# svenstaro/bvh

Measured on AMD Instinct MI355X. Metric: Mrays/s (build+traverse), higher is better.
Workload: dtype f32; 1 GPU; configs[1]: create_n_cubes(10000), 120000 triangles f32/3D, 1000000 create_ray rays per GPU; step = build_par+flatten+traverse; triangles=120000, rays_per_gpu=1000000, rays_total=1000000, scene_dist=single, flat_array=eager, parallelism=rays sharded x1

## Files before the change

### bvh_amd/csrc/traverse.hip

```cpp
#include <cstdio>
#include <type_traits>

#include "point_dist.hpp"
#include "walk.hpp"

namespace bvhgpu {

template <typename T, int MODE, bool STATS>
__global__ __launch_bounds__(256) void k_traverse(const TravNode<T>* __restrict__ nodes, uint32_t n_trav,
                                                  const typename Traits<T>::Ray* __restrict__ rays, uint32_t n_rays,
                                                  WalkOut<T> w) {
    const uint32_t r = blockIdx.x * blockDim.x + threadIdx.x;
    const int lane = lane_id();
    const unsigned long long lt = lanemask_lt();
    const bool active = r < n_rays;
    LaneRay<T, MODE> ray;
    ray.clear();
    if (active) ray.load(rays, r, w.tmax);
    uint32_t i = active ? 0u : n_trav;
    PoolCursor pc;
    unsigned long long steps = 0, leaf_steps = 0, wsteps = 0;
    const bool fast = MODE != MODE_T_SLICE && !__any(active && !ray.fin);
    while (true) {
        const bool run = i < n_trav;
// ... 118 lines not shown
    __device__ __forceinline__ void put(uint32_t e, T d, uint32_t n) {
        if (e < HEAP_LDS) { sd[e][tid] = d; sn[e][tid] = n; }
        else { gd[(size_t)(e - HEAP_LDS) * G + g] = d; gn[(size_t)(e - HEAP_LDS) * G + g] = n; }
    }
    __device__ __forceinline__ void sift_up(uint32_t pos, T d, uint32_t n) {
        while (pos > 0) {
            const uint32_t parent = (pos - 1) >> 1;
            const T pd = dist(parent);
            if (d <= pd) break;
            put(pos, pd, node(parent));
            pos = parent;
        }
        put(pos, d, n);
    }
};

template <typename T, int MODE, bool ASCENDING>
__global__ __launch_bounds__(256) void k_traverse_heap(const typename Traits<T>::Node* __restrict__ nodes, uint32_t n_nodes,
                                                       const T* __restrict__ shape_aabbs,
                                                       const typename Traits<T>::Ray* __restrict__ rays, uint32_t n_rays,
                                                       WalkOut<T> w, T* __restrict__ heap_dist, uint32_t* __restrict__ heap_node,
                                                       uint32_t heap_cap, uint32_t* __restrict__ overflow) {
    __shared__ T s_dist[HEAP_LDS][256];
    __shared__ uint32_t s_node[HEAP_LDS][256];
    const int lane = lane_id();
    const unsigned long long lt = lanemask_lt();
    LaneHeap<T> hp;
    hp.sd = s_dist; hp.sn = s_node; hp.gd = heap_dist; hp.gn = heap_node;
    hp.G = (size_t)gridDim.x * 256; hp.g = (size_t)blockIdx.x * 256 + threadIdx.x; hp.tid = threadIdx.x;
    const uint32_t cap = HEAP_LDS + heap_cap;
    PoolCursor pc;
    bool ovf = false;
    LaneRay<T, MODE> ray;
    for (size_t base = (size_t)blockIdx.x * 256; base < n_rays; base += hp.G) {
        const size_t r = base + threadIdx.x;
        const bool active = r < n_rays;
        ray.clear();
        if (active) ray.load(rays, (uint32_t)r);
        uint32_t len = 0;
        if (active && n_nodes) {
            bool has_node = true;
            const uint32_t rs = nodes[0].shape;
            if (rs != NONE) {
                const T* sb = shape_aabbs + 6 * (size_t)rs;
                const T mn[3] = {sb[0], sb[1], sb[2]}, mx[3] = {sb[3], sb[4], sb[5]};
                T t0, t1;
                has_node = slab_hit<T>(ray.o, ray.inv, mn, mx, t0, t1);
            }
            if (has_node) { hp.put(0, ASCENDING ? -(T)0 : (T)0, 0u); len = 1; }
        }
        while (true) {
            const bool run = len > 0;
            if (!__any(run)) break;
            bool rec = false;
            uint32_t shape = NONE;
            if (run) {
                len--;
                const T last_d = hp.dist(len);
                uint32_t node_index = hp.node(len);
                if (len > 0) {
                    const uint32_t last_n = node_index;
                    node_index = hp.node(0);
                    uint32_t pos = 0, child = 1;
                    while (child + 1 < len) {
                        T cd = hp.dist(child);
                        const T cr = hp.dist(child + 1);
                        if (cd <= cr) { child++; cd = cr; }
                        hp.put(pos, cd, hp.node(child));
                        pos = child;
                        child = 2 * pos + 1;
                    }
                    if (child == len - 1) { hp.put(pos, hp.dist(child), hp.node(child)); pos = child; }
                    hp.sift_up(pos, last_d, last_n);
                }
                const typename Traits<T>::Node* nd = nodes + node_index;
                const uint32_t ns = nd->shape;
                if (ns != NONE) {
                    rec = true; shape = ns;
                } else {
                    T lmn[3], lmx[3], rmn[3], rmx[3];
#pragma unroll
                    for (int k = 0; k < 3; k++) { lmn[k] = nd->l_min[k]; lmx[k] = nd->l_max[k]; rmn[k] = nd->r_min[k]; rmx[k] = nd->r_max[k]; }
                    const uint32_t li = nd->l, ri = nd->r;
                    T l0, l1, r0, r1;
                    const bool lh = slab_hit<T>(ray.o, ray.inv, lmn, lmx, l0, l1);
                    const bool rh = slab_hit<T>(ray.o, ray.inv, rmn, rmx, r0, r1);
                    if (len + (lh ? 1u : 0u) + (rh ? 1u : 0u) > cap) {
                        ovf = true; len = 0;
                    } else {
                        if (lh) { hp.sift_up(len, ASCENDING ? -l0 : l1, li); len++; }
                        if (rh) { hp.sift_up(len, ASCENDING ? -r0 : r1, ri); len++; }
                    }
                }
            }
            report<T, MODE>(rec, shape, (T)0, (T)0, ray, w, pc, lane, lt);
        }
        if (active) ray.retire(w);
    }
    if (ovf) atomicOr(overflow, HEAP_OVERFLOW_BIT);
    walk_epilogue<T, MODE>(w, pc, lane, false, 0, 0, 0, 0);
}

template <typename T> struct TopLds;
template <> struct TopLds<float> {
    static constexpr uint32_t BYTES_PER_SLOT = 32;
    float4 *lo, *hi;
    __device__ __forceinline__ TopLds(unsigned char* base, uint32_t K) {
        lo = reinterpret_cast<float4*>(base); hi = lo + K;
    }
    __device__ __forceinline__ void store(uint32_t q, const TravNode<float>* g) {
        const float4* p = reinterpret_cast<const float4*>(g);
        lo[q] = p[0]; hi[q] = p[1];
    }
    __device__ __forceinline__ NodeRegs<float> load(uint32_t q) const {
        const float4 a = lo[q], b = hi[q];
        NodeRegs<float> r;
        r.mn[0] = a.x; r.mn[1] = a.y; r.mn[2] = a.z; r.exit = __float_as_uint(a.w);
        r.mx[0] = b.x; r.mx[1] = b.y; r.mx[2] = b.z; r.shape = __float_as_uint(b.w);
        return r;
    }
};
template <> struct TopLds<double> {
    static constexpr uint32_t BYTES_PER_SLOT = 56;
    double2 *a, *b, *c;
    uint2* d;
    __device__ __forceinline__ TopLds(unsigned char* base, uint32_t K) {
        a = reinterpret_cast<double2*>(base); b = a + K; c = b + K; d = reinterpret_cast<uint2*>(c + K);
    }
    __device__ __forceinline__ void store(uint32_t q, const TravNode<double>* g) {
        const double2* p = reinterpret_cast<const double2*>(g);
        a[q] = p[0]; b[q] = p[1]; c[q] = p[2];
        const unsigned long long es = (unsigned long long)__double_as_longlong(p[3].x);
        d[q] = make_uint2((uint32_t)(es & 0xFFFFFFFFull), (uint32_t)(es >> 32));
    }
    __device__ __forceinline__ NodeRegs<double> load(uint32_t q) const {
        const double2 x = a[q], y = b[q], z = c[q];
        const uint2 w = d[q];
        NodeRegs<double> r;
        r.mn[0] = x.x; r.mn[1] = x.y; r.mn[2] = y.x;
        r.mx[0] = y.y; r.mx[1] = z.x; r.mx[2] = z.y;
        r.exit = w.x; r.shape = w.y;
        return r;
    }
};

constexpr int LDS_THREADS = 1024;
#ifndef BVH_LDS_INNER
#define BVH_LDS_INNER 8
#endif
constexpr int LDS_INNER = BVH_LDS_INNER;

template <typename T, int MODE, bool STATS>
__global__ __launch_bounds__(LDS_THREADS) void k_traverse_lds(const TravNode<T>* __restrict__ nodes, uint32_t n_trav,
                                                               const uint32_t* __restrict__ slot_entry, uint32_t K,
                                                               uint32_t first_slot, uint32_t split,
                                                               const typename Traits<T>::Ray* __restrict__ rays,
                                                               uint32_t n_rays, uint32_t rays_per_wg, WalkOut<T> w) {
    extern __shared__ __attribute__((aligned(16))) unsigned char smem[];
    uint32_t& s_next = *reinterpret_cast<uint32_t*>(smem);
    TopLds<T> top(smem + 16, K);
    const uint32_t split_at = split ? load_node(nodes).exit : 0u;
    const unsigned long long g0 = (unsigned long long)blockIdx.x * rays_per_wg;
    const unsigned long long g1 = g0 + rays_per_wg;
    const uint32_t wg_begin = (uint32_t)(g0 < n_rays ? g0 : n_rays);
    const uint32_t wg_end = (uint32_t)(g1 < n_rays ? g1 : n_rays);
    if (threadIdx.x == 0) s_next = wg_begin;
    for (uint32_t q = threadIdx.x; q < K; q += blockDim.x) {
        const uint32_t e = slot_entry[q];
        if (e != NONE) top.store(q, nodes + e);
    }
    __syncthreads();

    const int lane = lane_id();
    const unsigned long long lt = lanemask_lt();
    LaneRay<T, MODE> ray;
    ray.clear();
    uint32_t i = 0, limit = 0, slot = SLOT_NONE;
    bool exhausted = wg_begin >= wg_end;
    PoolCursor pc;
    unsigned long long steps = 0, leaf_steps = 0, wsteps = 0, cands = 0;
    while (true) {
        bool run = i < limit;
        const unsigned long long idle = __ballot(!run);
        if (idle) {
            if (!run && ray.r != NONE) { cands += ray.cnt; ray.retire(w); }
            if (!exhausted) {
                const uint32_t nidle = (uint32_t)__popcll(idle);
                uint32_t base = 0;
                if (lane == 0) base = atomicAdd(&s_next, nidle);
                base = __builtin_amdgcn_readfirstlane(base);
                const uint32_t mine = base + (uint32_t)__popcll(idle & lt);
                if (!run && base < wg_end && mine < wg_end) {
                    if (split_at) {
                        const bool right = (mine & 1u) != 0u;
                        ray.load(rays, mine >> 1, w.tmax);
                        ray.r = mine;
                        i = right ? split_at : 0u; limit = right ? n_trav : split_at;
                        slot = right ? 3u : 2u;
                    } else {
                        ray.load(rays, mine, w.tmax);
                        i = 0; limit = n_trav; slot = first_slot;
                    }
                    run = true;
                }
                exhausted = base >= wg_end || (wg_end - base) <= nidle;
            }
            if (!__any(run)) break;
        }
        const bool fast = MODE != MODE_T_SLICE && !__any(run && !ray.fin);
        for (int s = 0; s < LDS_INNER; s++) {
            bool rec = false;
            uint32_t shape = NONE;
            T t0 = 0, t1 = 0;
            if (STATS) wsteps++;
            if (i < limit) {
                NodeRegs<T> nd;
                if (slot < K) nd = top.load(slot);
                else nd = load_node(nodes + i);
                const bool hit = fast ? slab_hit_finite<T>(ray.o, ray.inv, nd.mn, nd.mx)
                                      : slab_hit<T>(ray.o, ray.inv, nd.mn, nd.mx, t0, t1);
                shape = nd.shape;
                const bool leaf = trav_is_leaf(shape);
                rec = hit && leaf;
                const bool descend = hit && !leaf;
                i = descend ? i + 1 : nd.exit;
                const uint32_t child = min(slot << 1, SLOT_NONE);
                slot = descend ? child : (leaf ? SLOT_NONE : (shape & 0xFFFFu));
                if (STATS) { steps++; leaf_steps += leaf ? 1 : 0; }
            }
            report<T, MODE>(rec, shape, t0, t1, ray, w, pc, lane, lt);
            if (MODE == MODE_ANY && ray.best_prim != NONE) i = limit;
        }
    }
    walk_epilogue<T, MODE>(w, pc, lane, STATS, steps, leaf_steps, wsteps, cands);
}

constexpr uint32_t CUR_NONE = 0x7FFFFFFFu;
#ifndef BVH_WIDE_INNER_STEPS
#define BVH_WIDE_INNER_STEPS 4
#endif
#ifndef BVH_WIDE_INNER_STEPS_WHOLE
#define BVH_WIDE_INNER_STEPS_WHOLE 8
#endif
#ifndef BVH_WIDE_INNER_STEPS_COHERENT
#define BVH_WIDE_INNER_STEPS_COHERENT 12
#endif
#ifndef BVH_WIDE_MIN_WAVES_F32
#define BVH_WIDE_MIN_WAVES_F32 8
#endif
#ifndef BVH_WIDE_MIN_WAVES_F64
#define BVH_WIDE_MIN_WAVES_F64 4
#endif
constexpr uint32_t WIDE_ITEM_BITS = 5;
constexpr uint32_t WIDE_ITEM_WHOLE = 16;
constexpr uint32_t WIDE_BSUM_MAX = 128;
constexpr size_t WIDE_ITEM_MAX_RAYS = (size_t)1 << 27;


__device__ __forceinline__ uint32_t wide_resident_ref(uint32_t ref, uint32_t q, uint32_t c, uint32_t K) {
    const uint32_t cs = 4u * q + 1u + c;
    return (ref != NONE && (ref & WIDE_INNER) && cs < K) ? (WIDE_INNER | WIDE_RESIDENT | cs) : ref;
}

template <typename T, bool EXACT>
__device__ __forceinline__ uint32_t wide_hits(const T o[3], const T inv[3], const WideRegs<T>& nd) {
    uint32_t m = 0;
    if (!EXACT) {
#pragma unroll
        for (int c = 0; c < 4; c++) {
            const T mn[3] = {nd.mn[0][c], nd.mn[1][c], nd.mn[2][c]}, mx[3] = {nd.mx[0][c], nd.mx[1][c], nd.mx[2][c]};
            m |= slab_hit_finite<T>(o, inv, mn, mx) ? (1u << c) : 0u;
        }
        return m;
    }
#pragma unroll
    for (int p = 0; p < 2; p++) {
        const int c0 = 2 * p, c1 = 2 * p + 1;
        const T mn0[3] = {nd.mn[0][c0], nd.mn[1][c0], nd.mn[2][c0]}, mx0[3] = {nd.mx[0][c0], nd.mx[1][c0], nd.mx[2][c0]};
        T t0, t1;
        if (nd.ref[c1] == NONE) {
            if (nd.ref[c0] != NONE && slab_hit<T>(o, inv, mn0, mx0, t0, t1)) m |= 1u << c0;
        } else {
            const T mn1[3] = {nd.mn[0][c1], nd.mn[1][c1], nd.mn[2][c1]}, mx1[3] = {nd.mx[0][c1], nd.mx[1][c1], nd.mx[2][c1]};
            T jmn[3], jmx[3];
#pragma unroll
            for (int k = 0; k < 3; k++) { jmn[k] = tmin(mn0[k], mn1[k]); jmx[k] = tmax(mx0[k], mx1[k]); }
            if (slab_hit<T>(o, inv, jmn, jmx, t0, t1)) {
                if (slab_hit<T>(o, inv, mn0, mx0, t0, t1)) m |= 1u << c0;
                if (slab_hit<T>(o, inv, mn1, mx1, t0, t1)) m |= 1u << c1;
            }
        }
    }
    return m;
}

#ifndef BVH_WIDE_LONG_FRAC
#define BVH_WIDE_LONG_FRAC 0.2
#endif
template <typename T> struct ItemTable {
    T box[16][6];
    uint32_t ref[16];
    T half_diag[16];
};
template <typename T, int ITEMS_LOG4>
__device__ __forceinline__ void item_table_build(const WideNode<T>* __restrict__ wide, ItemTable<T>* tb, uint32_t tid) {
    constexpr uint32_t ITEMS = 1u << (2 * ITEMS_LOG4);
    if (tid < ITEMS) {
        const uint32_t c = ITEMS_LOG4 == 2 ? tid >> 2 : tid, k = tid & 3u;
        const WideNode<T>* root = wide;
        uint32_t ref = root->ref[c];
        T b[6];
#pragma unroll
        for (int a = 0; a < 3; a++) { b[a] = root->mn[a][c]; b[3 + a] = root->mx[a][c]; }
        if (ITEMS_LOG4 == 2) {
            if (ref != NONE && (ref & WIDE_INNER)) {
                const WideNode<T>* g = wide + (ref & (WIDE_RESIDENT - 1u));
                ref = g->ref[k];
#pragma unroll
                for (int a = 0; a < 3; a++) { b[a] = g->mn[a][k]; b[3 + a] = g->mx[a][k]; }
            } else if (k != 0) {
                ref = NONE;
            }
        }
        if (ref == NONE) {
            const T nan = __builtin_nan("");
#pragma unroll
            for (int a = 0; a < 6; a++) b[a] = nan;
        }
#pragma unroll
        for (int a = 0; a < 6; a++) tb->box[tid][a] = b[a];
        tb->ref[tid] = ref;
        const T dx = b[3] - b[0], dy = b[4] - b[1], dz = b[5] - b[2];
        tb->half_diag[tid] = (T)BVH_WIDE_LONG_FRAC * sqrt(dx * dx + dy * dy + dz * dz);
    }
}
template <int ITEMS_LOG4> __device__ __forceinline__ uint32_t item_slot(uint32_t j) {
    return ITEMS_LOG4 == 2 ? 5u + j : 1u + j;
}

struct GuideArgs;
__device__ __forceinline__ void guide_ray_load(const bvhgpu_ray_f64* __restrict__ rays64, uint32_t r, double S, float o[3], float inv[3], bool& bad);
template <typename T, int L4, bool GUIDE = false>
__device__ __forceinline__ void filter_rays_into_list(const ItemTable<T>* tb, const typename Traits<T>::Ray* __restrict__ rays, uint32_t n_rays,
                                                      uint32_t* __restrict__ list, uint32_t per_wg, uint32_t my_rays, uint32_t G, uint32_t b,
                                                      uint32_t tid, uint32_t bd, int lane, uint32_t* s_nlist, uint32_t* s_nback,
                                                      const bvhgpu_ray_f64* __restrict__ rays64 = nullptr, double guide_S = 0.0, bool* any_bad = nullptr) {
    constexpr uint32_t ITEMS = 1u << (2 * L4);
    for (uint32_t l0 = 0; l0 < my_rays; l0 += bd) {
        const uint32_t local = l0 + tid;
        const uint32_t r = local < my_rays ? ((((local >> 6) * G + b) << 6) | (local & 63u)) : n_rays;
        uint32_t mask = 0, longm = 0;
        if (r < n_rays) {
            T o[3], inv[3];
            if constexpr (GUIDE) {
                bool bad;
                guide_ray_load(rays64, r, guide_S, o, inv, bad);
                *any_bad = *any_bad || bad;
            } else {
                const typename Traits<T>::Ray* rp = rays + r;
#pragma unroll
                for (int k = 0; k < 3; k++) { o[k] = rp->o[k]; inv[k] = rp->inv[k]; }
            }
            if (!ray_is_finite<T>(o, inv)) {
                mask = 1u << WIDE_ITEM_WHOLE; longm = mask;
            } else {
#pragma unroll 4
                for (uint32_t j = 0; j < ITEMS; j++) {
                    const T mn[3] = {tb->box[j][0], tb->box[j][1], tb->box[j][2]}, mx[3] = {tb->box[j][3], tb->box[j][4], tb->box[j][5]};
                    T len;
                    const bool hit = slab_hit_finite_len<T>(o, inv, mn, mx, len);
                    mask |= hit ? (1u << j) : 0u;
                    longm |= (hit && len > tb->half_diag[j]) ? (1u << j) : 0u;
                }
            }
        }
        const uint32_t cap = per_wg * ITEMS;
#pragma unroll
        for (int side = 0; side < 2; side++) {
            const uint32_t mm0 = side ? (mask & ~longm) : (mask & longm);
            const uint32_t mine = (uint32_t)__popc(mm0);
            uint32_t incl = mine;
#pragma unroll
            for (int d = 1; d < WAVE; d <<= 1) {
                const uint32_t u = __shfl_up(incl, d);
                if (lane >= d) incl += u;
            }
            const uint32_t total = __shfl(incl, WAVE - 1);
            uint32_t base = 0;
            if (lane == 0 && total) base = atomicAdd(side ? s_nback : s_nlist, total);
            base = __shfl(base, 0) + incl - mine;
            uint32_t mm = mm0;
            while (mm) {
                const uint32_t bit = (uint32_t)__ffs(mm) - 1u;
                mm &= mm - 1u;
                list[side ? cap - 1u - base : base] = (r << WIDE_ITEM_BITS) | bit;
                base++;
            }
        }
    }
}

template <typename T>
__global__ __launch_bounds__(256) void k_wide_items(const typename Traits<T>::Node* __restrict__ nodes, uint32_t n_nodes,
                                                    const uint32_t* __restrict__ node_count, const uint32_t* __restrict__ build_ctr,
                                                    const typename Traits<T>::Ray* __restrict__ rays, uint32_t n_rays,
                                                    uint32_t* __restrict__ list_all, uint32_t* __restrict__ wg_items) {
    constexpr int L4 = 2;
    constexpr uint32_t ITEMS = 16;
    __shared__ ItemTable<T> tb;
    __shared__ uint32_t s_nlist, s_nback, s_bad;
    const uint32_t tid = threadIdx.x, bd = blockDim.x;
    const int lane = lane_id();
    if (tid == 0) { s_nlist = 0u; s_nback = 0u; s_bad = (build_ctr[BUILD_CTR_TOPMASK] & 0xFFFEu) == 0xFFFEu ? 0u : 1u; }
    __syncthreads();
    if (s_bad) { if (tid == 0) wg_items[2u * blockIdx.x] = NONE; return; }
    if (tid < ITEMS) {
        uint32_t node = 0;
        T bx[6];
        bool ok = n_nodes > 1u;
        uint32_t cnt = ok ? node_count[0] : 0u;
#pragma unroll
        for (int lv = 3; lv >= 0 && ok; lv--) {
            const typename Traits<T>::Node nd = nodes[node];
            const uint32_t right = ((16u + tid) >> lv) & 1u;
            ok = nd.shape == NONE && nd.l < n_nodes && nd.r < n_nodes && nd.r > nd.l;
            if (!ok) break;
            const uint32_t nl = (nd.r - nd.l + 1u) >> 1;
            cnt = right ? cnt - nl : nl;
            node = right ? nd.r : nd.l;
#pragma unroll
            for (int k = 0; k < 3; k++) { bx[k] = right ? nd.r_min[k] : nd.l_min[k]; bx[3 + k] = right ? nd.r_max[k] : nd.l_max[k]; }
        }
        ok = ok && cnt > 1u;
        if (!ok) atomicOr(&s_bad, 1u);
#pragma unroll
        for (int k = 0; k < 6; k++) tb.box[tid][k] = bx[k];
        const T dx = bx[3] - bx[0], dy = bx[4] - bx[1], dz = bx[5] - bx[2];
        tb.half_diag[tid] = (T)BVH_WIDE_LONG_FRAC * sqrt(dx * dx + dy * dy + dz * dz);
    }
    __syncthreads();
    if (s_bad) { if (tid == 0) wg_items[2u * blockIdx.x] = NONE; return; }
    const uint32_t n_blocks = (n_rays + 63u) >> 6;
    const uint32_t my_blocks = n_blocks > blockIdx.x ? (n_blocks - blockIdx.x + gridDim.x - 1u) / gridDim.x : 0u;
    const uint32_t per_wg = ((n_blocks + gridDim.x - 1u) / gridDim.x) << 6;
    uint32_t* list = list_all + (size_t)blockIdx.x * per_wg * ITEMS;
    filter_rays_into_list<T, L4>(&tb, rays, n_rays, list, per_wg, my_blocks << 6, gridDim.x, blockIdx.x, tid, bd, lane, &s_nlist, &s_nback);
    __syncthreads();
    if (tid == 0) { wg_items[2u * blockIdx.x] = s_nlist; wg_items[2u * blockIdx.x + 1u] = s_nback; }
}

constexpr unsigned long long WALK_FLAG_GUIDE_RANGE = 16ull;
struct GuideArgs { const bvhgpu_ray_f64* rays64; const double* aabbs64; const float* info; const double* tris64; };
__device__ __forceinline__ void guide_ray_load(const bvhgpu_ray_f64* __restrict__ rays64, uint32_t r, double S, float o[3], float inv[3], bool& bad) {
    const bvhgpu_ray_f64* q = rays64 + r;
    bad = !(S >= GUIDE_SCENE_MIN) || !(S <= GUIDE_SCENE_MAX);
#pragma unroll
    for (int k = 0; k < 3; k++) {
        const double ok = q->o[k], ik = q->inv[k];
        const double ao = fabs(ok), ainv = fabs(ik), ai = ainv * (4.0 * S);
        bad = bad || !(ao <= GUIDE_ORIGIN_MAX * S) || !(ao <= GUIDE_F32_MAX) || !(ai <= 0x1p100) || !(ai >= 0x1p-100) ||
              !(ainv <= GUIDE_F32_MAX) || !(ainv >= GUIDE_F32_MIN_NORMAL);
        o[k] = (float)ok; inv[k] = (float)ik;
    }
}
__device__ __forceinline__ bool guide_leaf_hit(const GuideArgs& ga, uint32_t ray, uint32_t shape) {
    const bvhgpu_ray_f64* rp = ga.rays64 + ray;
    const double* b = ga.aabbs64 + 6 * (size_t)shape;
    const double o[3] = {rp->o[0], rp->o[1], rp->o[2]}, inv[3] = {rp->inv[0], rp->inv[1], rp->inv[2]};
    const double mn[3] = {b[0], b[1], b[2]}, mx[3] = {b[3], b[4], b[5]};
    return slab_hit_finite<double>(o, inv, mn, mx);
}

#ifndef BVH_GUIDE_CANDIDATE_ATTR
#define BVH_GUIDE_CANDIDATE_ATTR __forceinline__
#endif
__device__ BVH_GUIDE_CANDIDATE_ATTR double guide_candidate_distance(const bvhgpu_ray_f64* __restrict__ rays64, const double* __restrict__ tris64, uint32_t ray, uint32_t shape) {
    const bvhgpu_ray_f64* rp = rays64 + ray;
    const double o[3] = {rp->o[0], rp->o[1], rp->o[2]}, d[3] = {rp->d[0], rp->d[1], rp->d[2]};
    double out[3];
    ray_triangle<double>(o, d, tris64 + 9 * (size_t)shape, out);
    return out[0];
}

#ifdef BVH_WIDE_PROFILE
__device__ unsigned long long g_wide_prof[4 * 16384];
__device__ unsigned long long g_wide_util[16 * 16384];
#endif
template <typename T, int MODE, int ITEMS_LOG4, int MAX_THREADS, int MIN_WAVES, int GUIDE = 0>
__global__ __launch_bounds__(MAX_THREADS, MIN_WAVES) void k_traverse_wide(
    const WideNode<T>* __restrict__ wide, const uint32_t* __restrict__ wslot_node, uint32_t K, uint32_t stack_lds,
    const typename Traits<T>::Ray* __restrict__ rays, uint32_t n_rays, uint32_t* __restrict__ list_all, const uint32_t* __restrict__ wg_items,
    WalkOut<T> w, uint32_t* __restrict__ gstack, uint32_t gstack_cap, uint32_t* __restrict__ overflow, GuideArgs ga, uint32_t whole_steps) {
    static_assert(GUIDE == 0 || ((MODE == MODE_INDICES || MODE == MODE_CLOSEST) && sizeof(T) == 4), "the guide walk is the f32 walk of an f64 index / closest-hit batch");
    constexpr bool GUIDE_CLOSEST = GUIDE != 0 && MODE == MODE_CLOSEST;
    double gbest = 0.0;
    static_assert(ITEMS_LOG4 >= 0 && ITEMS_LOG4 <= 2, "1, 4 or 16 items per ray");
    static_assert(MODE != MODE_T_SLICE, "the t-slice output walks the binary array");
    constexpr int CH = WideIo<T>::CHUNKS;
    constexpr int L4 = ITEMS_LOG4 > 0 ? ITEMS_LOG4 : 1;
    constexpr uint32_t ITEMS = 1u << (2 * L4);
    extern __shared__ __attribute__((aligned(16))) uint4 wsmem[];
    uint32_t& s_next = *reinterpret_cast<uint32_t*>(wsmem);
    uint32_t& s_nlist = *(reinterpret_cast<uint32_t*>(wsmem) + 1);
    uint32_t& s_nback = *(reinterpret_cast<uint32_t*>(wsmem) + 2);
    uint32_t* s_item_ref = reinterpret_cast<uint32_t*>(wsmem + 1);
    uint4* nodes = wsmem + 5;
    uint32_t* s_stack = reinterpret_cast<uint32_t*>(nodes + (size_t)CH * K);
    const uint32_t bd = blockDim.x, tid = threadIdx.x;
    const int WIDE_INNER_STEPS = ITEMS_LOG4 == 0 ? (int)whole_steps : BVH_WIDE_INNER_STEPS;
    constexpr uint32_t SB = MAX_THREADS;
    const size_t G = (size_t)gridDim.x * bd, gid = (size_t)blockIdx.x * bd + tid;
    const int lane = lane_id();
    const unsigned long long lt = lanemask_lt();
    double guide_S = 0.0;
    bool guide_bad = false;
    if constexpr (GUIDE != 0) guide_S = (double)ga.info[0];
#ifdef BVH_WIDE_PROFILE
    const unsigned long long prof_t0 = wall_clock64();
    unsigned long long prof_steps = 0;
    unsigned long long pu[16];
    for (int i = 0; i < 16; i++) pu[i] = 0;
    uint32_t pl_boxes = 0, pl_nohit = 0;
#endif
    const uint32_t n_blocks = (n_rays + 63u) >> 6;
    const uint32_t my_blocks = n_blocks > blockIdx.x ? (n_blocks - blockIdx.x + gridDim.x - 1u) / gridDim.x : 0u;
    const uint32_t per_wg = ((n_blocks + gridDim.x - 1u) / gridDim.x) << 6;
    const uint32_t my_rays = my_blocks << 6;
    auto ray_of = [&](uint32_t local) -> uint32_t { return (((local >> 6) * gridDim.x + blockIdx.x) << 6) | (local & 63u); };
    __shared__ uint32_t s_bsum[WIDE_BSUM_MAX];
    if (w.scan_sums) for (uint32_t b = tid; b < WIDE_BSUM_MAX; b += bd) s_bsum[b] = 0u;
    if (tid == 0) { s_next = 0u; s_nlist = 0u; s_nback = 0u; }
    for (uint32_t q = tid; q < K; q += bd) {
        const uint32_t node = wslot_node[q];
        if (node != NONE) {
            const uint4* src = reinterpret_cast<const uint4*>(wide + node);
            uint4* dst = nodes + (size_t)q * CH;
#pragma unroll
            for (int c = 0; c < CH - 1; c++) dst[c] = src[c];
            uint4 rf = src[CH - 1];
            rf.x = wide_resident_ref(rf.x, q, 0u, K); rf.y = wide_resident_ref(rf.y, q, 1u, K);
            rf.z = wide_resident_ref(rf.z, q, 2u, K); rf.w = wide_resident_ref(rf.w, q, 3u, K);
            dst[CH - 1] = rf;
        }
    }
    uint32_t* list = nullptr;
    if (ITEMS_LOG4 > 0) {
        __shared__ ItemTable<T> tb;
        item_table_build<T, L4>(wide, &tb, tid);
        __syncthreads();
        if (tid < ITEMS) {
            const uint32_t ref = tb.ref[tid], slot = item_slot<L4>(tid);
            s_item_ref[tid] = (ref != NONE && (ref & WIDE_INNER) && slot < K) ? (WIDE_INNER | WIDE_RESIDENT | slot) : ref;
        }
        list = list_all + (size_t)blockIdx.x * per_wg * ITEMS;
        const uint32_t pre_front = wg_items ? wg_items[2u * blockIdx.x] : NONE;
        if (pre_front != NONE) {
            if (tid == 0) { s_nlist = pre_front; s_nback = wg_items[2u * blockIdx.x + 1u]; }
        } else {
            if constexpr (GUIDE != 0) filter_rays_into_list<T, L4, true>(&tb, rays, n_rays, list, per_wg, my_rays, gridDim.x, blockIdx.x, tid, bd, lane, &s_nlist, &s_nback,
                                                                            ga.rays64, guide_S, &guide_bad);
            else filter_rays_into_list<T, L4>(&tb, rays, n_rays, list, per_wg, my_rays, gridDim.x, blockIdx.x, tid, bd, lane, &s_nlist, &s_nback);
        }
        __threadfence_block();
    }
    __syncthreads();
    const uint32_t wg_begin = 0u;
    const uint32_t n_front = s_nlist;
    const uint32_t wg_end = ITEMS_LOG4 == 0 ? my_rays : n_front + s_nback;
#ifdef BVH_WIDE_PROFILE
    const unsigned long long prof_t1 = wall_clock64();
#endif

    LaneRay<T, MODE> ray;
    ray.clear();
    uint32_t cur = CUR_NONE, sp = 0, item = NONE;
    bool exhausted = wg_begin >= wg_end;
    bool ovf = false;
    uint32_t pair_pend = NONE;
    PoolCursor pc;
    auto push_slow = [&](uint32_t v) {
        if (sp < stack_lds) s_stack[sp * SB + tid] = v;
        else if (sp - stack_lds < gstack_cap) gstack[(size_t)(sp - stack_lds) * G + gid] = v;
        else ovf = true;
        sp++;
    };
    auto pop_or_none = [&]() -> uint32_t {
        if (sp == 0) return CUR_NONE;
        sp--;
        if (sp < stack_lds) return s_stack[sp * SB + tid];
        return sp - stack_lds < gstack_cap ? gstack[(size_t)(sp - stack_lds) * G + gid] : CUR_NONE;
    };
    while (true) {
        bool run = cur != CUR_NONE;
        const unsigned long long idle = __ballot(!run);
        if (idle) {
            if (MODE == MODE_INDICES && ITEMS_LOG4 == 0 && w.pool_pair)
                report_pair(false, !run && item != NONE, 0u, ray, pair_pend, w.pool_pair, w.pool_cap, w.ctr, pc, lane, lt);
            if (!run && item != NONE) {
                if (MODE == MODE_ANY) {
                    if constexpr (ITEMS_LOG4 == 0) {
                        const size_t r = item;
                        w.closest[3 * r] = ray.best[0]; w.closest[3 * r + 1] = ray.best[1]; w.closest[3 * r + 2] = ray.best[2];
                        w.closest_prim[r] = ray.best_prim;
                    } else if (ray.best_prim != NONE) {
                        const uint32_t j = item & ((1u << WIDE_ITEM_BITS) - 1u);
                        const uint32_t jj = j == WIDE_ITEM_WHOLE ? 0u : j;
                        atomicMin(&w.any_key[item >> WIDE_ITEM_BITS], (jj << 28) | ray.best_prim);
                    }
                } else if (MODE == MODE_CLOSEST) {
                    if constexpr (ITEMS_LOG4 == 0) {
                        const size_t r = item;
                        if constexpr (!GUIDE_CLOSEST) { w.closest[3 * r] = ray.best[0]; w.closest[3 * r + 1] = ray.best[1]; w.closest[3 * r + 2] = ray.best[2]; }
                        w.closest_prim[r] = ray.best_prim;
                    } else if (ray.best_prim != NONE) {
                        const uint32_t j = item & ((1u << WIDE_ITEM_BITS) - 1u);
                        const uint32_t jj = j == WIDE_ITEM_WHOLE ? 0u : j;
                        if constexpr (sizeof(T) == 4 && !GUIDE_CLOSEST) {
                            const unsigned long long key = ((unsigned long long)Traits<T>::key(ray.best[0]) << 32) | ((unsigned long long)jj << 28) | (unsigned long long)ray.best_prim;
                            atomicMin(&w.closest_key[item >> WIDE_ITEM_BITS], key);
                        } else {
                            const size_t r = item >> WIDE_ITEM_BITS;
                            w.item_cnt[(r << (2 * ITEMS_LOG4)) + jj] = ray.best_prim;
                            atomicOr(&w.ray_items[r], 1u << jj);
                        }
                    }
                } else if (ray.cnt) {
                    uint32_t r = item;
                    if (ITEMS_LOG4 == 0) {
                        w.counts[item] = ray.cnt;
                    } else {
                        const uint32_t j = item & ((1u << WIDE_ITEM_BITS) - 1u);
                        const uint32_t jj = j == WIDE_ITEM_WHOLE ? 0u : j;
                        r = item >> WIDE_ITEM_BITS;
                        atomicAdd(&w.counts[r], ray.cnt);
                        atomicOr(&w.ray_items[r], 1u << jj);
                        w.item_cnt[((size_t)r << (2 * ITEMS_LOG4)) + jj] = ray.cnt;
                    }
                    if (w.scan_sums) atomicAdd(&s_bsum[((r >> 6) - blockIdx.x) / gridDim.x], ray.cnt);
                }
                item = NONE;
            }
            if (!exhausted) {
                const uint32_t nidle = (uint32_t)__popcll(idle);
                uint32_t base = 0;
                if (lane == 0) base = atomicAdd(&s_next, nidle);
                base = __builtin_amdgcn_readfirstlane(base);
                const uint32_t mine = base + (uint32_t)__popcll(idle & lt);
                if (!run && base < wg_end && mine < wg_end) {
                    if (ITEMS_LOG4 == 0) {
                        item = ray_of(mine);
                        if (item < n_rays) {
                            if constexpr (GUIDE != 0) { bool bad; guide_ray_load(ga.rays64, item, guide_S, ray.o, ray.inv, bad); guide_bad = guide_bad || bad; ray.loaded(item); gbest = __builtin_inf(); }
                            else ray.load(rays, item, w.tmax);
                            cur = WIDE_INNER | WIDE_RESIDENT | 0u;
                        } else {
                            item = NONE;
                        }
                    } else {
                        item = list[mine < n_front ? mine : per_wg * ITEMS - 1u - (mine - n_front)];
                        const uint32_t j = item & ((1u << WIDE_ITEM_BITS) - 1u);
                        if constexpr (GUIDE != 0) { bool bad; guide_ray_load(ga.rays64, item >> WIDE_ITEM_BITS, guide_S, ray.o, ray.inv, bad); ray.loaded(item >> WIDE_ITEM_BITS); gbest = __builtin_inf(); }
                        else ray.load(rays, item >> WIDE_ITEM_BITS, w.tmax);
                        cur = j == WIDE_ITEM_WHOLE ? (WIDE_INNER | WIDE_RESIDENT | 0u) : s_item_ref[j];
                        if (j == WIDE_ITEM_WHOLE) item = item & ~((1u << WIDE_ITEM_BITS) - 1u);
                    }
                    ray.r = item;
                    sp = 0;
                    run = cur != CUR_NONE;
                }
                exhausted = base >= wg_end || (wg_end - base) <= nidle;
            }
            if (!__any(run)) break;
        }
        const bool fast = !__any(run && !ray.fin);
#ifdef BVH_WIDE_PROFILE
        prof_steps += WIDE_INNER_STEPS;
        pu[9]++; pu[10] += fast ? 0 : 1;
        pu[8] += WIDE_INNER_STEPS * (unsigned long long)__popcll(__ballot(run));
#endif
        for (int s = 0; s < WIDE_INNER_STEPS; s++) {
#ifdef BVH_WIDE_PROFILE
            {
                const bool in = (cur & WIDE_INNER) != 0u;
                pu[0]++; pu[1] += __popcll(__ballot(in));
                pu[2] += __any(in && (cur & WIDE_RESIDENT)) ? 1 : 0;
                pu[3] += __any(in && !(cur & WIDE_RESIDENT)) ? 1 : 0;
                const bool slow = in && sp + 3u > stack_lds;
                pu[4] += __any(slow) ? 1 : 0; pu[5] += __popcll(__ballot(slow));
                const bool lf = !in && cur < CUR_NONE;
                pu[6] += __popcll(__ballot(lf)); pu[7] += __any(lf) ? 1 : 0;
                pu[11] += __any((in || lf) && sp > stack_lds) ? 1 : 0;
            }
#endif
            if (cur & WIDE_INNER) {
                const uint32_t id = cur & (WIDE_RESIDENT - 1u);
                WideRegs<T> nd;
                if (cur & WIDE_RESIDENT) nd = WideIo<T>::from_lds(nodes, id);
                else nd = WideIo<T>::from_global(wide + id);
                const uint32_t m = fast ? wide_hits<T, false>(ray.o, ray.inv, nd) : wide_hits<T, true>(ray.o, ray.inv, nd);
                const uint32_t first = m & (0u - m);
                const uint32_t rest = m ^ first;
#ifdef BVH_WIDE_PROFILE
                pl_boxes += (uint32_t)__popc(m); pl_nohit += m == 0u ? 1u : 0u;
#endif
                const uint32_t s0 = (rest & 8u) ? nd.ref[3] : ((rest & 4u) ? nd.ref[2] : nd.ref[1]);
                const uint32_t s1 = ((rest & 12u) == 12u) ? nd.ref[2] : nd.ref[1];
                if (sp + 3u <= stack_lds) {
                    uint32_t* at = s_stack + sp * SB + tid;
                    at[0] = s0; at[SB] = s1; at[2 * SB] = nd.ref[1];
                    sp += (uint32_t)__popc(rest);
                } else {
                    if (rest & 8u) push_slow(nd.ref[3]);
                    if (rest & 4u) push_slow(nd.ref[2]);
                    if (rest & 2u) push_slow(nd.ref[1]);
                }
                cur = first == 0u ? pop_or_none() : (first == 1u ? nd.ref[0] : (first == 2u ? nd.ref[1] : (first == 4u ? nd.ref[2] : nd.ref[3])));
            }
            bool rec = cur < CUR_NONE;
            const uint32_t shape = cur;
            if (rec) cur = pop_or_none();
            if (GUIDE) {
                if (__any(rec)) {
                    if (rec) rec = guide_leaf_hit(ga, ITEMS_LOG4 == 0 ? ray.r : (ray.r >> WIDE_ITEM_BITS), shape);
                }
            }
            if (MODE == MODE_INDICES && ITEMS_LOG4 == 0 && w.raybuf) {
                if (rec && (ray.cnt >> w.stage_shift) == 0u) {
                    w.raybuf[((size_t)ray.r << w.stage_shift) | ray.cnt] = shape;
                    ray.cnt++;
                    rec = false;
                }
            }
            if constexpr (GUIDE_CLOSEST) {
                if (__any(rec)) {
                    if (rec) {
                        const double dist = guide_candidate_distance(ga.rays64, ga.tris64, ITEMS_LOG4 == 0 ? ray.r : (ray.r >> WIDE_ITEM_BITS), shape);
                        if (dist < gbest) { gbest = dist; ray.best_prim = shape; }
                        ray.cnt++;
                    }
                }
            } else if (MODE == MODE_INDICES && ITEMS_LOG4 == 0 && w.pool_pair) report_pair(rec, false, shape, ray, pair_pend, w.pool_pair, w.pool_cap, w.ctr, pc, lane, lt);
            else report<T, MODE>(rec, shape, (T)0, (T)0, ray, w, pc, lane, lt);
            if (MODE == MODE_ANY && ray.best_prim != NONE) { cur = CUR_NONE; sp = 0; }
        }
        if (ovf) { cur = CUR_NONE; sp = 0; }
    }
    if (__any(ovf) && lane == 0) atomicOr(overflow, 4u);
    if constexpr (GUIDE != 0) { if (__any(guide_bad) && lane == 0) atomicOr(overflow, (uint32_t)WALK_FLAG_GUIDE_RANGE); }
    if (MODE == MODE_INDICES && ITEMS_LOG4 == 0 && w.pool_pair) {
        pool_invalidate_tail16(w.pool_pair, w.pool_cap, pc, lane);
        pc.left = 0;
    }
    walk_epilogue<T, MODE>(w, pc, lane, false, 0, 0, 0, 0);
    if (MODE < MODE_CLOSEST && w.scan_sums) {
        __syncthreads();
        for (uint32_t b = tid; b < my_blocks; b += bd)
            if (s_bsum[b]) atomicAdd(&w.scan_sums[(b * gridDim.x + blockIdx.x) / (uint32_t)(SCAN_BLOCK / 64)], s_bsum[b]);
    }
#ifdef BVH_WIDE_PROFILE
    if (lane == 0) {
        const size_t wv = gid >> 6;
        if (wv < 16384) {
            g_wide_prof[4 * wv] = prof_t0; g_wide_prof[4 * wv + 1] = prof_t1; g_wide_prof[4 * wv + 2] = wall_clock64(); g_wide_prof[4 * wv + 3] = prof_steps;
            for (int i = 0; i < 12; i++) g_wide_util[16 * wv + i] = pu[i];
            g_wide_util[16 * wv + 12] = 0; g_wide_util[16 * wv + 13] = 0;
        }
    }
    __syncthreads();
    if ((gid >> 6) < 16384) { atomicAdd(&g_wide_util[16 * (gid >> 6) + 12], (unsigned long long)pl_boxes); atomicAdd(&g_wide_util[16 * (gid >> 6) + 13], (unsigned long long)pl_nohit); }
#endif
}


constexpr int COUNT_PLAIN = 0, COUNT_PAIR = 1, COUNT_MASKED = 2;
template <int KIND> __device__ __forceinline__ uint32_t ray_count(const uint32_t* __restrict__ counts, uint32_t r) {
    if (KIND == COUNT_PLAIN || KIND == COUNT_MASKED) return counts[r];
    const uint2 c = reinterpret_cast<const uint2*>(counts)[r];
    return c.x + c.y;
}

template <int KIND>
__global__ __launch_bounds__(256) void k_scan_reduce(const uint32_t* __restrict__ counts, uint32_t n,
                                                     unsigned long long* __restrict__ blocksums) {
    __shared__ unsigned long long ws[4];
    const uint32_t base = blockIdx.x * SCAN_BLOCK + threadIdx.x * SCAN_ITEMS;
    unsigned long long s = 0;
#pragma unroll
    for (int j = 0; j < SCAN_ITEMS; j++) s += (base + j < n) ? ray_count<KIND>(counts, base + j) : 0u;
#pragma unroll
    for (int d = 32; d > 0; d >>= 1) s += __shfl_down(s, d);
    if (lane_id() == 0) ws[threadIdx.x >> 6] = s;
    __syncthreads();
    if (threadIdx.x == 0) blocksums[blockIdx.x] = ws[0] + ws[1] + ws[2] + ws[3];
}

__global__ __launch_bounds__(1024) void k_scan_sums(unsigned long long* __restrict__ blocksums, uint32_t nb,
                                                    unsigned long long* __restrict__ total_out) {
    __shared__ unsigned long long ws[16];
    const uint32_t per = (nb + 1023u) / 1024u;
    const uint32_t lo = min(nb, threadIdx.x * per), hi = min(nb, lo + per);
    unsigned long long s = 0;
    for (uint32_t j = lo; j < hi; j++) s += blocksums[j];
    const int lane = lane_id(), wv = (int)(threadIdx.x >> 6);
    unsigned long long inc = s;
#pragma unroll
    for (int d = 1; d < WAVE; d <<= 1) {
        const unsigned long long u = __shfl_up(inc, d);
        if (lane >= d) inc += u;
    }
    if (lane == WAVE - 1) ws[wv] = inc;
    __syncthreads();
    unsigned long long run = inc - s;
    for (int w2 = 0; w2 < wv; w2++) run += ws[w2];
    for (uint32_t j = lo; j < hi; j++) { const unsigned long long v = blocksums[j]; blocksums[j] = run; run += v; }
    if (threadIdx.x == 1023u) *total_out = run;
}

constexpr uint32_t SCAN_FUSED_MAX_BLOCKS = 2048;

template <int KIND, bool PREFIXED>
__global__ __launch_bounds__(256) void k_scan_final(const uint32_t* __restrict__ counts, uint32_t n,
                                                    const unsigned long long* __restrict__ blocksums,
                                                    unsigned long long* __restrict__ total,
                                                    uint32_t* __restrict__ offsets, uint32_t* __restrict__ ray_items,
                                                    uint16_t* __restrict__ ray_mask, unsigned long long* __restrict__ host_page,
                                                    unsigned long long* __restrict__ other_ctr, const uint32_t* __restrict__ scan_sums,
                                                    uint32_t* __restrict__ other_bsum, uint32_t bsum_cap) {
    __shared__ uint32_t ws[4];
    __shared__ unsigned long long wb[4];
    const uint32_t base = blockIdx.x * SCAN_BLOCK + threadIdx.x * SCAN_ITEMS;
    const int lane = lane_id();
    unsigned long long before = 0;
    if (PREFIXED) {
        before = blocksums[blockIdx.x];
    } else {
        unsigned long long part = 0;
        if (scan_sums) {
            for (uint32_t j = threadIdx.x; j < blockIdx.x; j += 256) part += scan_sums[j];
            if (threadIdx.x == 0) other_bsum[blockIdx.x] = 0u;
            if (blockIdx.x == gridDim.x - 1)
                for (uint32_t j = gridDim.x + threadIdx.x; j < bsum_cap; j += 256) other_bsum[j] = 0u;
        } else {
            for (uint32_t j = threadIdx.x; j < blockIdx.x; j += 256) part += blocksums[j];
        }
#pragma unroll
        for (int d = 32; d > 0; d >>= 1) part += __shfl_down(part, d);
        if (lane == 0) wb[threadIdx.x >> 6] = part;
    }
    uint32_t v[SCAN_ITEMS];
    uint32_t s = 0;
#pragma unroll
    for (int j = 0; j < SCAN_ITEMS; j++) { v[j] = (base + j < n) ? ray_count<KIND>(counts, base + j) : 0u; s += v[j]; }
    if (KIND == COUNT_MASKED) {
#pragma unroll
        for (int j = 0; j < SCAN_ITEMS; j++) {
            if (v[j]) {
                if (ray_items) { ray_mask[base + j] = (uint16_t)ray_items[base + j]; ray_items[base + j] = 0u; }
                const_cast<uint32_t*>(counts)[base + j] = 0u;
            }
        }
    }
    uint32_t inc = s;
#pragma unroll
    for (int d = 1; d < WAVE; d <<= 1) {
// ... 1108 lines not shown
```

Before: 3006 Mrays/s.

## Overlap wide-node image copy, item table loads, and ray prefetch in traversal prologue

Splits the item-table build into separate root and grandchild issue phases and interleaves them with a batched copy of resident wide nodes into the node image. Each thread now holds several uint4 chunks in registers before storing them. The first ray of the filter pass is loaded early, and the filter loop prefetches the next round's ray while processing the current one. The goal is to hide global-memory latency in the kernel prologue, at the cost of more live registers, which may lower occupancy.

```diff
diff --git a/bvh_amd/csrc/traverse.hip b/bvh_amd/csrc/traverse.hip
--- a/bvh_amd/csrc/traverse.hip
+++ b/bvh_amd/csrc/traverse.hip
@@ -444,37 +444,40 @@
     uint32_t ref[16];
     T half_diag[16];
 };
+template <typename T> struct ItemEntry { T b[6]; uint32_t ref; };
 template <typename T, int ITEMS_LOG4>
-__device__ __forceinline__ void item_table_build(const WideNode<T>* __restrict__ wide, ItemTable<T>* tb, uint32_t tid) {
-    constexpr uint32_t ITEMS = 1u << (2 * ITEMS_LOG4);
-    if (tid < ITEMS) {
-        const uint32_t c = ITEMS_LOG4 == 2 ? tid >> 2 : tid, k = tid & 3u;
-        const WideNode<T>* root = wide;
-        uint32_t ref = root->ref[c];
-        T b[6];
-#pragma unroll
-        for (int a = 0; a < 3; a++) { b[a] = root->mn[a][c]; b[3 + a] = root->mx[a][c]; }
-        if (ITEMS_LOG4 == 2) {
-            if (ref != NONE && (ref & WIDE_INNER)) {
-                const WideNode<T>* g = wide + (ref & (WIDE_RESIDENT - 1u));
-                ref = g->ref[k];
-#pragma unroll
-                for (int a = 0; a < 3; a++) { b[a] = g->mn[a][k]; b[3 + a] = g->mx[a][k]; }
-            } else if (k != 0) {
-                ref = NONE;
-            }
-        }
-        if (ref == NONE) {
-            const T nan = __builtin_nan("");
-#pragma unroll
-            for (int a = 0; a < 6; a++) b[a] = nan;
-        }
-#pragma unroll
-        for (int a = 0; a < 6; a++) tb->box[tid][a] = b[a];
-        tb->ref[tid] = ref;
-        const T dx = b[3] - b[0], dy = b[4] - b[1], dz = b[5] - b[2];
-        tb->half_diag[tid] = (T)BVH_WIDE_LONG_FRAC * sqrt(dx * dx + dy * dy + dz * dz);
-    }
+__device__ __forceinline__ void item_table_issue_root(const WideNode<T>* __restrict__ wide, ItemEntry<T>& e, uint32_t tid) {
+    const uint32_t c = ITEMS_LOG4 == 2 ? tid >> 2 : tid;
+    e.ref = wide->ref[c];
+#pragma unroll
+    for (int a = 0; a < 3; a++) { e.b[a] = wide->mn[a][c]; e.b[3 + a] = wide->mx[a][c]; }
+}
+template <typename T, int ITEMS_LOG4>
+__device__ __forceinline__ void item_table_issue_grand(const WideNode<T>* __restrict__ wide, ItemEntry<T>& e, uint32_t tid) {
+    if (ITEMS_LOG4 == 2) {
+        const uint32_t k = tid & 3u;
+        if (e.ref != NONE && (e.ref & WIDE_INNER)) {
+            const WideNode<T>* g = wide + (e.ref & (WIDE_RESIDENT - 1u));
+            e.ref = g->ref[k];
+#pragma unroll
+            for (int a = 0; a < 3; a++) { e.b[a] = g->mn[a][k]; e.b[3 + a] = g->mx[a][k]; }
+        } else if (k != 0) {
+            e.ref = NONE;
+        }
+    }
+}
+template <typename T>
+__device__ __forceinline__ void item_table_store(ItemEntry<T>& e, ItemTable<T>* tb, uint32_t tid) {
+    if (e.ref == NONE) {
+        const T nan = __builtin_nan("");
+#pragma unroll
+        for (int a = 0; a < 6; a++) e.b[a] = nan;
+    }
+#pragma unroll
+    for (int a = 0; a < 6; a++) tb->box[tid][a] = e.b[a];
+    tb->ref[tid] = e.ref;
+    const T dx = e.b[3] - e.b[0], dy = e.b[4] - e.b[1], dz = e.b[5] - e.b[2];
+    tb->half_diag[tid] = (T)BVH_WIDE_LONG_FRAC * sqrt(dx * dx + dy * dy + dz * dz);
 }
 template <int ITEMS_LOG4> __device__ __forceinline__ uint32_t item_slot(uint32_t j) {
     return ITEMS_LOG4 == 2 ? 5u + j : 1u + j;
@@ -482,15 +485,43 @@
 
 struct GuideArgs;
 __device__ __forceinline__ void guide_ray_load(const bvhgpu_ray_f64* __restrict__ rays64, uint32_t r, double S, float o[3], float inv[3], bool& bad);
-template <typename T, int L4, bool GUIDE = false>
+template <typename T> struct FilterRay {
+    T o[3], inv[3];
+    __device__ __forceinline__ void request(const typename Traits<T>::Ray* __restrict__ rays, uint32_t r, uint32_t n_rays) {
+#pragma unroll
+        for (int k = 0; k < 3; k++) { o[k] = 0; inv[k] = 0; }
+        if (r < n_rays) {
+            const typename Traits<T>::Ray* rp = rays + r;
+#pragma unroll
+            for (int k = 0; k < 3; k++) { o[k] = rp->o[k]; inv[k] = rp->inv[k]; }
+        }
+    }
+};
+template <typename T, int L4, bool GUIDE>
 __device__ __forceinline__ void filter_rays_into_list(const ItemTable<T>* tb, const typename Traits<T>::Ray* __restrict__ rays, uint32_t n_rays,
                                                       uint32_t* __restrict__ list, uint32_t per_wg, uint32_t my_rays, uint32_t G, uint32_t b,
                                                       uint32_t tid, uint32_t bd, int lane, uint32_t* s_nlist, uint32_t* s_nback,
-                                                      const bvhgpu_ray_f64* __restrict__ rays64 = nullptr, double guide_S = 0.0, bool* any_bad = nullptr) {
+                                                      const bvhgpu_ray_f64* __restrict__ rays64, double guide_S, bool* any_bad,
+                                                      bool have_first, const FilterRay<T>& first) {
     constexpr uint32_t ITEMS = 1u << (2 * L4);
+    auto ray_of_round = [&](uint32_t l0) -> uint32_t {
+        const uint32_t local = l0 + tid;
+        return local < my_rays ? ((((local >> 6) * G + b) << 6) | (local & 63u)) : n_rays;
+    };
+    FilterRay<T> cur_ray, next_ray;
+    uint32_t r = ray_of_round(0u);
+    if constexpr (!GUIDE) {
+        if (have_first) cur_ray = first;
+        else cur_ray.request(rays, r, n_rays);
+    }
     for (uint32_t l0 = 0; l0 < my_rays; l0 += bd) {
-        const uint32_t local = l0 + tid;
-        const uint32_t r = local < my_rays ? ((((local >> 6) * G + b) << 6) | (local & 63u)) : n_rays;
+        uint32_t r_next = n_rays;
+        if constexpr (!GUIDE) {
+            if (l0 + bd < my_rays) r_next = ray_of_round(l0 + bd);
+            next_ray.request(rays, r_next, n_rays);
+        } else {
+            r = ray_of_round(l0);
+        }
         uint32_t mask = 0, longm = 0;
         if (r < n_rays) {
             T o[3], inv[3];
@@ -499,9 +530,8 @@
                 guide_ray_load(rays64, r, guide_S, o, inv, bad);
                 *any_bad = *any_bad || bad;
             } else {
-                const typename Traits<T>::Ray* rp = rays + r;
-#pragma unroll
-                for (int k = 0; k < 3; k++) { o[k] = rp->o[k]; inv[k] = rp->inv[k]; }
+#pragma unroll
+                for (int k = 0; k < 3; k++) { o[k] = cur_ray.o[k]; inv[k] = cur_ray.inv[k]; }
             }
             if (!ray_is_finite<T>(o, inv)) {
                 mask = 1u << WIDE_ITEM_WHOLE; longm = mask;
@@ -539,7 +569,16 @@
                 base++;
             }
         }
-    }
+        if constexpr (!GUIDE) { r = r_next; cur_ray = next_ray; }
+    }
+}
+template <typename T, int L4>
+__device__ __forceinline__ void filter_rays_into_list(const ItemTable<T>* tb, const typename Traits<T>::Ray* __restrict__ rays, uint32_t n_rays,
+                                                      uint32_t* __restrict__ list, uint32_t per_wg, uint32_t my_rays, uint32_t G, uint32_t b,
+                                                      uint32_t tid, uint32_t bd, int lane, uint32_t* s_nlist, uint32_t* s_nback) {
+    FilterRay<T> none;
+    none.request(rays, n_rays, n_rays);
+    filter_rays_into_list<T, L4, false>(tb, rays, n_rays, list, per_wg, my_rays, G, b, tid, bd, lane, s_nlist, s_nback, nullptr, 0.0, nullptr, false, none);
 }
 
 template <typename T>
@@ -670,38 +709,90 @@
     const uint32_t my_rays = my_blocks << 6;
     auto ray_of = [&](uint32_t local) -> uint32_t { return (((local >> 6) * gridDim.x + blockIdx.x) << 6) | (local & 63u); };
     __shared__ uint32_t s_bsum[WIDE_BSUM_MAX];
+    constexpr bool OWN_ITEMS = ITEMS_LOG4 > 0;
+    const bool ray_first = OWN_ITEMS && GUIDE == 0 && wg_items == nullptr;
+    FilterRay<T> first_ray;
+    first_ray.request(rays, ray_first && tid < my_rays ? ray_of(tid) : n_rays, n_rays);
+    uint32_t pre_front = NONE, pre_back = 0u;
+    if (OWN_ITEMS && wg_items) { pre_front = wg_items[2u * blockIdx.x]; pre_back = wg_items[2u * blockIdx.x + 1u]; }
+    constexpr int IMG = sizeof(T) == 8 ? 8 : 4;
+    const uint32_t img_total = K * (uint32_t)CH;
+    uint32_t img_node[IMG];
+    uint4 img_v[IMG];
+    auto image_request_nodes = [&](uint32_t e0) {
+#pragma unroll
+        for (int i = 0; i < IMG; i++) {
+            const uint32_t e = e0 + (uint32_t)i * bd;
+            img_node[i] = e < img_total ? wslot_node[e / (uint32_t)CH] : NONE;
+        }
+    };
+    auto image_request_chunks = [&](uint32_t e0) {
+#pragma unroll
+        for (int i = 0; i < IMG; i++) {
+            const uint32_t e = e0 + (uint32_t)i * bd;
+            img_v[i] = reinterpret_cast<const uint4*>(wide + (img_node[i] != NONE ? img_node[i] : 0u))[e % (uint32_t)CH];
+        }
+    };
+    auto image_store = [&](uint32_t e0) {
+#pragma unroll
+        for (int i = 0; i < IMG; i++) {
+            const uint32_t e = e0 + (uint32_t)i * bd, q = e / (uint32_t)CH;
+            if (img_node[i] != NONE) {
+                uint4 v = img_v[i];
+                if (e - q * (uint32_t)CH == (uint32_t)CH - 1u) {
+                    v.x = wide_resident_ref(v.x, q, 0u, K); v.y = wide_resident_ref(v.y, q, 1u, K);
+                    v.z = wide_resident_ref(v.z, q, 2u, K); v.w = wide_resident_ref(v.w, q, 3u, K);
+                }
+                nodes[e] = v;
+            }
+        }
+    };
+    __shared__ ItemTable<T> tb;
+    ItemEntry<T> item_entry;
+    if constexpr (OWN_ITEMS) {
+        image_request_nodes(tid);
+        if (tid < ITEMS) item_table_issue_root<T, L4>(wide, item_entry, tid);
+    }
     if (w.scan_sums) for (uint32_t b = tid; b < WIDE_BSUM_MAX; b += bd) s_bsum[b] = 0u;
-    if (tid == 0) { s_next = 0u; s_nlist = 0u; s_nback = 0u; }
-    for (uint32_t q = tid; q < K; q += bd) {
-        const uint32_t node = wslot_node[q];
-        if (node != NONE) {
-            const uint4* src = reinterpret_cast<const uint4*>(wide + node);
-            uint4* dst = nodes + (size_t)q * CH;
-#pragma unroll
-            for (int c = 0; c < CH - 1; c++) dst[c] = src[c];
-            uint4 rf = src[CH - 1];
-            rf.x = wide_resident_ref(rf.x, q, 0u, K); rf.y = wide_resident_ref(rf.y, q, 1u, K);
-            rf.z = wide_resident_ref(rf.z, q, 2u, K); rf.w = wide_resident_ref(rf.w, q, 3u, K);
-            dst[CH - 1] = rf;
+    if (tid == 0) { s_next = 0u; s_nlist = pre_front != NONE ? pre_front : 0u; s_nback = pre_front != NONE ? pre_back : 0u; }
+    if constexpr (OWN_ITEMS) {
+        image_request_chunks(tid);
+        if (tid < ITEMS) item_table_issue_grand<T, L4>(wide, item_entry, tid);
+        image_store(tid);
+        for (uint32_t e0 = tid + (uint32_t)IMG * bd; e0 < img_total; e0 += (uint32_t)IMG * bd) {
+            image_request_nodes(e0);
+            image_request_chunks(e0);
+            image_store(e0);
+        }
+    } else {
+        for (uint32_t q = tid; q < K; q += bd) {
+            const uint32_t node = wslot_node[q];
+            if (node != NONE) {
+                const uint4* src = reinterpret_cast<const uint4*>(wide + node);
+                uint4* dst = nodes + (size_t)q * CH;
+#pragma unroll
+                for (int c = 0; c < CH - 1; c++) dst[c] = src[c];
+                uint4 rf = src[CH - 1];
+                rf.x = wide_resident_ref(rf.x, q, 0u, K); rf.y = wide_resident_ref(rf.y, q, 1u, K);
+                rf.z = wide_resident_ref(rf.z, q, 2u, K); rf.w = wide_resident_ref(rf.w, q, 3u, K);
+                dst[CH - 1] = rf;
+            }
         }
     }
     uint32_t* list = nullptr;
-    if (ITEMS_LOG4 > 0) {
-        __shared__ ItemTable<T> tb;
-        item_table_build<T, L4>(wide, &tb, tid);
+    if (OWN_ITEMS) {
+        if (tid < ITEMS) {
+            item_table_store<T>(item_entry, &tb, tid);
+            const uint32_t ref = item_entry.ref, slot = item_slot<L4>(tid);
+            s_item_ref[tid] = (ref != NONE && (ref & WIDE_INNER) && slot < K) ? (WIDE_INNER | WIDE_RESIDENT | slot) : ref;
+        }
         __syncthreads();
-        if (tid < ITEMS) {
-            const uint32_t ref = tb.ref[tid], slot = item_slot<L4>(tid);
-            s_item_ref[tid] = (ref != NONE && (ref & WIDE_INNER) && slot < K) ? (WIDE_INNER | WIDE_RESIDENT | slot) : ref;
-        }
         list = list_all + (size_t)blockIdx.x * per_wg * ITEMS;
-        const uint32_t pre_front = wg_items ? wg_items[2u * blockIdx.x] : NONE;
-        if (pre_front != NONE) {
-            if (tid == 0) { s_nlist = pre_front; s_nback = wg_items[2u * blockIdx.x + 1u]; }
-        } else {
+        if (pre_front == NONE) {
             if constexpr (GUIDE != 0) filter_rays_into_list<T, L4, true>(&tb, rays, n_rays, list, per_wg, my_rays, gridDim.x, blockIdx.x, tid, bd, lane, &s_nlist, &s_nback,
-                                                                            ga.rays64, guide_S, &guide_bad);
-            else filter_rays_into_list<T, L4>(&tb, rays, n_rays, list, per_wg, my_rays, gridDim.x, blockIdx.x, tid, bd, lane, &s_nlist, &s_nback);
+                                                                            ga.rays64, guide_S, &guide_bad, false, first_ray);
+            else filter_rays_into_list<T, L4, false>(&tb, rays, n_rays, list, per_wg, my_rays, gridDim.x, blockIdx.x, tid, bd, lane, &s_nlist, &s_nback,
+                                                     nullptr, 0.0, nullptr, ray_first, first_ray);
         }
         __threadfence_block();
     }
```

Result: no change. 2987 Mrays/s (-0.6%).
